# jianglab/helicon

Measured on NVIDIA B200. Metric: denovo3D candidates/sec (solve+score), higher is better.
Workload: dtype f32 (u,v,h) / f64 (x,hbar; bounded branch), as scipy executes it

## Files before the change

helicon_b200/csrc/hb2_api.cu:

```cuda
#include "../../include/helicon_b200.h"
#include "hb2_kernels.cuh"
#include "hb2_trf.cuh"
#include "hb2_symm.cuh"
#include "hb2_tie.cuh"
#include "hb2_fwd_band.cuh"
#include "hb2_adj_tile.cuh"
#include "hb2_explicit.cuh"
#include "hb2_bilinear.cuh"

#include <cub/cub.cuh>
#include <nvtx3/nvToolsExt.h>

#include <algorithm>
#include <cstdio>
#include <cstring>
#include <cstdlib>
#include <string>
#include <vector>

struct NvtxRange {
  explicit NvtxRange(const char* name) { nvtxRangePushA(name); }
  ~NvtxRange() { nvtxRangePop(); }
  NvtxRange(const NvtxRange&) = delete;
  NvtxRange& operator=(const NvtxRange&) = delete;
// ... 190 lines not shown
  float* d_ls_w = nullptr;
  uint16_t* d_amap_i = nullptr;
  bool bilinear = false;
  int bil_nM = 0;
  std::vector<uint8_t> h_bil_rv;
  std::vector<int> h_bil_view_map, h_bil_colk, h_bil_cand_nview;
  std::vector<double> h_bil_ab;
  std::vector<int2*> ls_ent_c;
  std::vector<int> ls_m_c;
  struct LsScratch {
    long long cap_rows = 0, sort_cap = 0;
    int pairs_cap = 0;
    LsymPair* pairs = nullptr;
    unsigned long long *tab_key = nullptr, *tab_seq = nullptr;
    int *tmp_a = nullptr, *tmp_b = nullptr, *flag = nullptr, *pos = nullptr, *ov = nullptr;
    void* scan_tmp = nullptr; size_t scan_bytes = 0;
    int *col = nullptr; float* w = nullptr;
    int *key = nullptr, *key2 = nullptr, *id = nullptr, *id2 = nullptr, *cc = nullptr;
    void* sort_tmp = nullptr; size_t sort_bytes = 0;
  } ls_scr;
  long long extra_launches = 0;
  int max_views = 0;
  bool created = false;
  int nviews = 0;
  std::vector<hb2_candidate> cands;
  std::vector<int> h_view_count, h_view_begin, h_mdata, h_msym;
  std::vector<long long> h_uoff, h_symoff, h_symcap, h_cscoff;
  std::vector<int> tie_per_angle;
  std::vector<int> h_view_angle;
  std::vector<double> h_cs;
  std::vector<uint32_t> cand_flags;
  long long u_total = 0;
  double* d_cs = nullptr;
  void* d_fmap = nullptr;
  uint8_t* d_rayvalid = nullptr;
  int* d_tie = nullptr;
  uint16_t* d_amap = nullptr;
  int* d_sym_g = nullptr;
  std::vector<std::vector<int>> h_sym_round_end;
  int* d_sym_a = nullptr; int* d_sym_b = nullptr; int* d_csc_ptr = nullptr; int* d_csc_ent = nullptr; int* d_ell = nullptr;
  float* d_bmax = nullptr;
  float* d_score = nullptr;
  float* d_chain = nullptr;
  int* d_nactive = nullptr;
  int* h_nactive = nullptr;
  double timing[16] = {0};
  std::vector<TrfState> last_trf;
  std::vector<cudaEvent_t> ev_pool;
  std::vector<std::pair<int, int>> ev_used;
  size_t ev_next = 0;
  bool profiling = false;
  bool solved = false;
  cudaStream_t side = nullptr;
  cudaEvent_t ev_fork = nullptr, ev_join = nullptr;
};

extern "C" const char* hb2_last_error(void) { return g_err.c_str(); }
extern "C" int hb2_device_count(void) {
  int n = 0;
  if (cudaGetDeviceCount(&n) != cudaSuccess) { cudaGetLastError(); return 0; }
  return n;
}
extern "C" const char* hb2_build_info(void) { return "helicon_b200 sm_100a " __DATE__ " " __TIME__; }

extern "C" int hb2_stream_create(int device, void** out) {
  if (!out) return fail(HB2_ERR_ARG, "null argument");
  if (hb2_device_count() <= 0) return fail(HB2_ERR_NO_DEVICE, "no CUDA device visible; helicon_b200 has no CPU fallback");
  CK(cudaSetDevice(device));
  cudaStream_t st;
  CK(cudaStreamCreateWithFlags(&st, cudaStreamNonBlocking));
  *out = (void*)st;
  return HB2_OK;
}
extern "C" int hb2_stream_destroy(int device, void* stream) {
  if (!stream) return HB2_OK;
  CK(cudaSetDevice(device));
  CK(cudaStreamSynchronize((cudaStream_t)stream));
  {
    std::lock_guard<std::mutex> lk(g_arena_mu);
    auto it = g_arenas.find({device, (cudaStream_t)stream});
    if (it != g_arenas.end() && it->second->live == 0) {
      if (it->second->base) cudaFree(it->second->base);
      delete it->second;
      g_arenas.erase(it);
    }
  }
  CK(cudaStreamDestroy((cudaStream_t)stream));
  return HB2_OK;
}
extern "C" int hb2_device_trim(int device) {
  if (hb2_device_count() <= 0) return HB2_OK;
  CK(cudaSetDevice(device));
  CK(cudaDeviceSynchronize());
  std::lock_guard<std::mutex> lk(g_arena_mu);
  for (auto& kv : g_arenas) {
    Arena* a = kv.second;
    if (kv.first.first == device && a->live == 0 && a->base) { cudaFree(a->base); a->base = nullptr; a->cap = 0; a->top = 0; }
  }
  return HB2_OK;
}

static void disk_tables(int G, double rmin, int rmax, std::vector<int>& rank, std::vector<short2>& yx) {
  rank.assign((size_t)G * G, -1);
  yx.clear();
  int c0 = G / 2;
  for (int y = 0; y < G; ++y)
// ... 1447 lines not shown
  ~ProfScope() {
    if (!b->profiling) return;
    cudaEventRecord(b->ev_pool[first + 1], s);
  }
};

static void launch_fwd_data(hb2_batch* b, int mode) {
  ProfScope ps(b, KC_FWD_DATA);
  const BD& B = b->B;
  cudaStream_t st = b->stream;
  if (b->nviews == 0) return;
  if (b->n_tie_views > 0) {
    const float* src = mode == MODE_LSMR ? B.v : B.xs;
    if (b->bilinear) {
      const dim3 gv(b->n_tie_views, B.fwd_ppv);
#define FBIL(I, Q) k_fwd_bil<I, Q, float, false><<<gv, HB2_BLOCK, 0, st>>>(B, TD{}, src, B.u, mode)
#define FBILQ(I) do { if (B.L3P == 4) FBIL(I, 1); else if (B.L3P == 8) FBIL(I, 2); else if (B.L3P == 12) FBIL(I, 3); else FBIL(I, 4); } while (0)
      if (b->idx16) FBILQ(uint16_t); else FBILQ(uint32_t);
#undef FBILQ
#undef FBIL
      k_fwd_lsym<float, false><<<gv, HB2_BLOCK, 0, st>>>(B, TD{}, src, B.u, mode);
      b->extra_launches += 1;
    } else if (b->explicit_rows) k_fwd_csr<float, false><<<dim3(b->n_tie_views, B.fwd_ppv), HB2_BLOCK, 0, st>>>(B, TD{}, src, B.u, mode);
    else if (b->idx16) k_fwd_tie<uint16_t, float, false><<<dim3(b->n_tie_views, B.fwd_ppv), HB2_BLOCK, 0, st>>>(B, TD{}, src, B.u, mode);
    else k_fwd_tie<uint32_t, float, false><<<dim3(b->n_tie_views, B.fwd_ppv), HB2_BLOCK, 0, st>>>(B, TD{}, src, B.u, mode);
    b->extra_launches += 1;
  }
  if (B.fwd_band) {
    const size_t sm = b->fwd_band_smem;
    const dim3 gb(B.bt32.nband, B.nc), gr(b->max_views, B.nc);
#define FWB(Q)                                                                                            \
  do {                                                                                                    \
    hb2_allow_big_smem((const void*)k_fwd_band<Q, float, false>);                                         \
    k_fwd_band<Q, float, false><<<gb, HB2_FWDB_THREADS, sm, st>>>(B, TD{}, nullptr, mode);                \
    k_fwd_band_reduce<Q, float, false><<<gr, HB2_BLOCK, 0, st>>>(B, TD{}, nullptr, mode);                 \
  } while (0)
    if (B.L3P == 4) FWB(1); else if (B.L3P == 8) FWB(2); else if (B.L3P == 12) FWB(3); else FWB(4);
    b->extra_launches += 1;
#undef FWB
    return;
  }
  const int ntiles = (B.D2 + HB2_TILE_RAYS - 1) / HB2_TILE_RAYS;
  unsigned grid = (unsigned)b->nviews * ntiles;
#define FWD(T)                                                                              \
  do {                                                                                      \
    if (B.L3P == 4) k_fwd_data<T, 1><<<grid, HB2_BLOCK, 0, st>>>(B, mode);                  \
    else if (B.L3P == 8) k_fwd_data<T, 2><<<grid, HB2_BLOCK, 0, st>>>(B, mode);             \
    else if (B.L3P == 12) k_fwd_data<T, 3><<<grid, HB2_BLOCK, 0, st>>>(B, mode);            \
    else k_fwd_data<T, 4><<<grid, HB2_BLOCK, 0, st>>>(B, mode);                             \
  } while (0)
  if (b->idx16) FWD(uint16_t); else FWD(uint32_t);
#undef FWD
}
static void launch_fwd_sym(hb2_batch* b, int mode, cudaStream_t on = nullptr) {
  ProfScope ps(b, KC_FWD_SYM, on);
  const BD& B = b->B;
  dim3 g(B.part_us_per_cand, B.nc);
  k_fwd_sym<<<g, HB2_BLOCK, 0, on ? on : b->stream>>>(B, mode);
}
static void launch_adj(hb2_batch* b, int mode) {
  ProfScope ps(b, KC_ADJ);
  const BD& B = b->B;
  dim3 g(B.part_v_per_cand, B.nc);
  cudaStream_t st = b->stream;
  if (b->n_tie_views > 0) {
    if (b->bilinear) {
      const dim3 ga(cdiv(B.ndisk, (HB2_BLOCK / 32) * (32 / (B.L3P / 4))), B.nc);
      const size_t smt = (size_t)HB2_BILT_NS * HB2_BILT_SV * ((size_t)B.bil_KB * HB2_BLOCK * 6 + (size_t)B.bil_rmax * B.L3P * sizeof(float));
      const bool use_tile = B.bil_adj_tile && smt <= 200 * 1024;
#define ABIL(Q)                                                                                      \
  do {                                                                                               \
    k_bil_unblend<Q, float, false><<<b->n_tie_views, HB2_BLOCK, 0, st>>>(B, TD{}, B.u, B.bil_ub, mode); \
    if (use_tile && B.bil_KB == 3) {                                                                 \
      hb2_allow_big_smem((const void*)k_adj_bil_tile<Q, 3, float, false>);                           \
      k_adj_bil_tile<Q, 3, float, false><<<dim3(B.ntile, B.nc), HB2_BILT_THREADS, smt, st>>>(B, TD{}, B.bil_ub, B.vtie, mode); \
    } else if (use_tile) {                                                                           \
      hb2_allow_big_smem((const void*)k_adj_bil_tile<Q, 0, float, false>);                           \
      k_adj_bil_tile<Q, 0, float, false><<<dim3(B.ntile, B.nc), HB2_BILT_THREADS, smt, st>>>(B, TD{}, B.bil_ub, B.vtie, mode); \
    } else k_adj_bil<Q, float, false><<<ga, HB2_BLOCK, 0, st>>>(B, TD{}, B.bil_ub, B.vtie, mode);   \
  } while (0)
      if (B.L3P == 4) ABIL(1); else if (B.L3P == 8) ABIL(2); else if (B.L3P == 12) ABIL(3); else ABIL(4);
#undef ABIL
      k_adj_lsym<float, false><<<dim3(cdiv(B.npad, HB2_BLOCK), B.nc), HB2_BLOCK, 0, st>>>(B, TD{}, B.u, B.vtie, mode);
      b->extra_launches += 2;
    } else if (b->explicit_rows) k_adj_csc<float, false><<<dim3(cdiv(B.npad, HB2_BLOCK / 32), B.nc), HB2_BLOCK, 0, st>>>(B, TD{}, B.u, B.vtie, mode);
    else k_adj_tie<float, false><<<dim3(cdiv(B.ndisk, HB2_BLOCK), B.nc), HB2_BLOCK, 0, st>>>(B, TD{}, B.u, B.vtie, mode);
    b->extra_launches += 1;
  }
  if (B.adj_tile == 2) {
    const size_t sm = b->adj_tile_smem;
    const dim3 gc(B.ntile, B.nc, b->adj_chunks);
#define ADJTC(K)                                                                                                        \
  do {                                                                                                                  \
    hb2_allow_big_smem((const void*)k_adj_tile<4, K, float, false, true>);   \
    k_adj_tile<4, K, float, false, true><<<gc, HB2_ADJT_THREADS, sm, st>>>(B, TD{}, B.u, nullptr, mode);                \
  } while (0)
    if (B.K == 1) ADJTC(1); else ADJTC(2);
#undef ADJTC
    return;
  }
  if (B.adj_tile) {
    const size_t sm = b->adj_tile_smem;
#define ADJT(Q, K)                                                                                                   \
  do {                                                                                                               \
    hb2_allow_big_smem((const void*)k_adj_tile<Q, K, float, false>);      \
    k_adj_tile<Q, K, float, false><<<g, HB2_ADJT_THREADS, sm, st>>>(B, TD{}, B.u, nullptr, mode);                    \
  } while (0)
#define ADJTQ(K) do { if (B.L3P == 4) ADJT(1, K); else if (B.L3P == 8) ADJT(2, K); else if (B.L3P == 12) ADJT(3, K); else ADJT(4, K); } while (0)
    if (B.K == 1) ADJTQ(1); else ADJTQ(2);
#undef ADJTQ
#undef ADJT
    return;
  }
  if (B.adj_fast) {
    if (B.K == 1) k_adj_pq<1><<<g, HB2_BLOCK, 0, st>>>(B, mode);
    else k_adj_pq<2><<<g, HB2_BLOCK, 0, st>>>(B, mode);
    return;
  }
#define ADJ(K, M) k_adj<K, M><<<g, HB2_BLOCK, 0, st>>>(B, mode)
  if (B.MC == 1) ADJ(0, 1);
  else ADJ(0, 0);
#undef ADJ
}
static void launch_update(hb2_batch* b, int mode) {
  ProfScope ps(b, KC_UPDATE);
  const BD& B = b->B;
  dim3 g(B.part_x_per_cand, B.nc);
  k_update<<<g, HB2_BLOCK, 0, b->stream>>>(B, mode);
}

extern "C" int hb2_batch_apply_forward(hb2_batch* b, int32_t c, const float* x_host, float* y_host) {
  if (!b || !b->created || !x_host || !y_host || c < 0 || c >= b->B.nc) return fail(HB2_ERR_ARG, "bad argument");
  CK(cudaSetDevice(b->P->device));
  BD& B = b->B;
  cudaStream_t st = b->stream;
  long long m = (long long)b->h_mdata[c] + b->h_msym[c];
  std::vector<float> xi((size_t)B.npad, 0.f);
  for (int z = 0; z < B.L3; ++z)
    for (int pp = 0; pp < B.ndisk; ++pp) xi[(size_t)pp * B.L3P + z] = x_host[(size_t)z * B.ndisk + b->P->int2ref[pp]];
  CK(cudaMemcpyAsync(B.xs + (size_t)c * B.npad, xi.data(), sizeof(float) * B.npad, cudaMemcpyHostToDevice, st));
  CK(cudaMemsetAsync(B.u + b->h_uoff[c], 0, sizeof(float) * m, st));
  B.only_cand = c;
  launch_fwd_data(b, MODE_PLAIN);
  launch_fwd_sym(b, MODE_PLAIN);
  B.only_cand = -1;
  CKL();
  CK(cudaMemcpyAsync(y_host, B.u + b->h_uoff[c], sizeof(float) * m, cudaMemcpyDeviceToHost, st));
  CK(cudaStreamSynchronize(st));
  b->solved = false;
  return HB2_OK;
}

extern "C" int hb2_batch_apply_adjoint(hb2_batch* b, int32_t c, const float* y_host, float* x_host) {
  if (!b || !b->created || !x_host || !y_host || c < 0 || c >= b->B.nc) return fail(HB2_ERR_ARG, "bad argument");
  CK(cudaSetDevice(b->P->device));
  BD& B = b->B;
  cudaStream_t st = b->stream;
  long long m = (long long)b->h_mdata[c] + b->h_msym[c];
  CK(cudaMemcpyAsync(B.u + b->h_uoff[c], y_host, sizeof(float) * m, cudaMemcpyHostToDevice, st));
  B.only_cand = c;
  launch_adj(b, MODE_PLAIN);
  B.only_cand = -1;
  CKL();
  std::vector<float> xi((size_t)B.npad);
  CK(cudaMemcpyAsync(xi.data(), B.xs + (size_t)c * B.npad, sizeof(float) * B.npad, cudaMemcpyDeviceToHost, st));
  CK(cudaStreamSynchronize(st));
  for (int z = 0; z < B.L3; ++z)
    for (int pp = 0; pp < B.ndisk; ++pp) x_host[(size_t)z * B.ndisk + b->P->int2ref[pp]] = xi[(size_t)pp * B.L3P + z];
  b->solved = false;
  return HB2_OK;
}


static int run_trf(hb2_batch* b, const hb2_solve_options* opt, std::vector<TrfState>& out, long long& launches, int& outer_iters) {
  BD& B = b->B;
  cudaStream_t st = b->stream;
  const int nc = B.nc;
  bool any = false;
  for (int c = 0; c < nc; ++c) any = any || b->cands[c].positive;
  out.assign(nc, TrfState{});
  if (!any) return HB2_OK;
// ... 172 lines not shown
  }
  pass(OPC(EW_FINAL));
#undef OPC
  CKT2(cudaGetLastError());
  CKT2(cudaMemcpyAsync(out.data(), T.st, sizeof(TrfState) * nc, cudaMemcpyDeviceToHost, st));
  CKT2(cudaStreamSynchronize(st));
  tmp.free_all();
  B.vtie64 = nullptr;
  return HB2_OK;
}

extern "C" int hb2_batch_solve(hb2_batch* b, const hb2_solve_options* opt, hb2_result* res) {
  if (!b || !b->created || !opt || !res) return fail(HB2_ERR_ARG, "bad argument");
  CK(cudaSetDevice(b->P->device));
  NvtxRange nvtx_("solve_equations + score (batch)");
  nvtxRangePushA("solve_equations: LSMR");
  struct PopGuard { int n = 1; ~PopGuard() { while (n-- > 0) nvtxRangePop(); } } nvtx_stage_;
  BD& B = b->B;
  cudaStream_t st = b->stream;
  const int nc = B.nc;
  const int maxit = opt->max_iter > 0 ? opt->max_iter : 1000;
  const int check = opt->check_every > 0 ? opt->check_every : 8;
  B.clip_pred = opt->clip_pred;
  B.only_cand = -1;
  b->profiling = opt->profile != 0;
  b->ev_used.clear();
  b->ev_next = 0;
  cudaEvent_t e0, e1, e2;
  CK(cudaEventCreate(&e0)); CK(cudaEventCreate(&e1)); CK(cudaEventCreate(&e2));
  CK(cudaEventRecord(e0, st));
  size_t nv = (size_t)nc * B.npad;
  CK(cudaMemsetAsync(B.x, 0, nv * sizeof(double), st));
  CK(cudaMemsetAsync(B.hbar, 0, nv * sizeof(double), st));
  CK(cudaMemsetAsync(B.h, 0, nv * sizeof(float), st));
  CK(cudaMemsetAsync(B.v, 0, nv * sizeof(float), st));
  CK(cudaMemcpyAsync(B.u, B.b, sizeof(float) * (size_t)b->u_total, cudaMemcpyDeviceToDevice, st));
  CK(cudaMemsetAsync(b->d_nactive, 0, sizeof(int), st));
  long long launches = 0;
  b->extra_launches = 0;
  static const int env_norm = [] { const char* e = getenv("HB2_NORM_MODE"); return e ? atoi(e) : -1; }();
  const bool chain = (env_norm >= 0 ? env_norm : opt->norm_mode) != 0;
  if (chain) {
    hb2_allow_big_smem((const void*)k_chain_sumsq<CHAIN_U>);
    hb2_allow_big_smem((const void*)k_chain_sumsq<CHAIN_V>);
    hb2_allow_big_smem((const void*)k_chain_sumsq<CHAIN_B>);
  }
  float* ch_u = chain ? b->d_chain : nullptr;
  float* ch_v = chain ? b->d_chain + nc : nullptr;
  if (chain) { k_chain_sumsq<CHAIN_B><<<nc, 64, HB2_CHAIN_SMEM, st>>>(B, ch_u, MODE_INIT); ++launches; }
  k_scal_normb<<<nc, HB2_BLOCK, 0, st>>>(B, ch_u);
  launch_adj(b, MODE_INIT);
  if (chain) { k_chain_sumsq<CHAIN_V><<<nc, 64, HB2_CHAIN_SMEM, st>>>(B, ch_v, MODE_INIT); ++launches; }
  k_scal_init<<<nc, HB2_BLOCK, 0, st>>>(B, b->d_nactive, ch_v);
  launch_update(b, MODE_INIT);
  launches += 4;
  CKL();
  int it = 0;
  static const int env_overlap = [] { const char* e = getenv("HB2_OVERLAP"); return e ? atoi(e) : 1; }();
  const bool overlap = env_overlap != 0 && !b->profiling;
  if (overlap && !b->side) {
    CK(cudaStreamCreateWithFlags(&b->side, cudaStreamNonBlocking));
    CK(cudaEventCreateWithFlags(&b->ev_fork, cudaEventDisableTiming));
    CK(cudaEventCreateWithFlags(&b->ev_join, cudaEventDisableTiming));
  }
  *b->h_nactive = 1;
  CK(cudaMemcpyAsync(b->h_nactive, b->d_nactive, sizeof(int), cudaMemcpyDeviceToHost, st));
  CK(cudaStreamSynchronize(st));
  while (*b->h_nactive > 0 && it < maxit) {
    int burst = std::min(check, maxit - it);
    for (int q = 0; q < burst; ++q) {
      if (overlap) {
        cudaEventRecord(b->ev_fork, st);
        launch_fwd_data(b, MODE_LSMR);
        cudaStreamWaitEvent(b->side, b->ev_fork, 0);
        launch_fwd_sym(b, MODE_LSMR, b->side);
        cudaEventRecord(b->ev_join, b->side);
        cudaStreamWaitEvent(st, b->ev_join, 0);
      } else {
        launch_fwd_data(b, MODE_LSMR);
        launch_fwd_sym(b, MODE_LSMR);
      }
      if (chain) { ProfScope ps(b, KC_NORM); k_chain_sumsq<CHAIN_U><<<nc, 64, HB2_CHAIN_SMEM, st>>>(B, ch_u, MODE_LSMR); ++launches; }
      { ProfScope ps(b, KC_SCALAR); k_scal_beta<<<nc, HB2_BLOCK, 0, st>>>(B, ch_u); }
      launch_adj(b, MODE_LSMR);
      if (chain) { ProfScope ps(b, KC_NORM); k_chain_sumsq<CHAIN_V><<<nc, 64, HB2_CHAIN_SMEM, st>>>(B, ch_v, MODE_LSMR); ++launches; }
      { ProfScope ps(b, KC_SCALAR); k_scal_rot<<<nc, HB2_BLOCK, 0, st>>>(B, ch_v); }
      launch_update(b, MODE_LSMR);
      { ProfScope ps(b, KC_SCALAR); k_scal_test<<<nc, HB2_BLOCK, 0, st>>>(B, opt->atol, opt->btol, opt->conlim, maxit, opt->fixed_iters, b->d_nactive); }
      launches += 7;
    }
    it += burst;
    CKL();
    CK(cudaMemcpyAsync(b->h_nactive, b->d_nactive, sizeof(int), cudaMemcpyDeviceToHost, st));
    CK(cudaStreamSynchronize(st));
  }
  CK(cudaEventRecord(e1, st));
  std::vector<TrfState> trf;
  int trf_outer = 0;
  cudaEvent_t e1b;
  CK(cudaEventCreate(&e1b));
  {
    dim3 g(cdiv(B.npad, 256), nc);
    k_x_to_f32<<<g, 256, 0, st>>>(B);
    ++launches;
  }
  nvtxRangePop(); nvtxRangePushA("solve_equations: bounded TRF");
  if (opt->fixed_iters <= 0) {
    int rc = run_trf(b, opt, trf, launches, trf_outer);
    if (rc != HB2_OK) return rc;
  } else trf.assign(nc, TrfState{});
  CK(cudaEventRecord(e1b, st));
  nvtxRangePop(); nvtxRangePushA("cosine_similarity (reprojection + score)");
  {
    launch_fwd_data(b, MODE_SCORE);
    k_scal_score<<<nc, HB2_BLOCK, 0, st>>>(B, b->d_score);
    launches += 2;
    CKL();
  }
  CK(cudaEventRecord(e2, st));
  std::vector<LsmrState> hs(nc);
  std::vector<float> sc(nc);
  CK(cudaMemcpyAsync(hs.data(), B.st, sizeof(LsmrState) * nc, cudaMemcpyDeviceToHost, st));
  CK(cudaMemcpyAsync(sc.data(), b->d_score, sizeof(float) * nc, cudaMemcpyDeviceToHost, st));
  CK(cudaStreamSynchronize(st));
  float ms_l = 0, ms_s = 0, ms_t = 0;
  cudaEventElapsedTime(&ms_l, e0, e1); cudaEventElapsedTime(&ms_t, e1, e1b); cudaEventElapsedTime(&ms_s, e1b, e2);
  cudaEventDestroy(e0); cudaEventDestroy(e1); cudaEventDestroy(e1b); cudaEventDestroy(e2);
  for (double& t : b->timing) t = 0;
  b->timing[0] = ms_l; b->timing[1] = ms_t; b->timing[2] = ms_s; b->timing[13] = trf_outer; b->timing[3] = (double)(launches + b->extra_launches); b->timing[4] = it;
  if (b->profiling) {
    for (auto& pr : b->ev_used) {
      float ms = 0;
      cudaEventElapsedTime(&ms, b->ev_pool[pr.second], b->ev_pool[pr.second + 1]);
      if (pr.first == KC_NORM) b->timing[14] += ms;
      else b->timing[5 + pr.first] += ms;
      if (pr.first == KC_FWD_DATA) b->timing[10] += 1;
      if (pr.first == KC_ADJ) b->timing[11] += 1;
      if (pr.first == KC_UPDATE) b->timing[12] += 1;
    }
    b->profiling = false;
  }
  for (int c = 0; c < nc; ++c) {
    hb2_result& r = res[c];
// ... 319 lines not shown
```

helicon_b200/csrc/hb2_kernels.cuh:

```cuda
#pragma once
#include "hb2_common.cuh"

#define HB2_MAX_ZMC 1024
#define HB2_TILE_RAYS 32
#define HB2_BLOCK 256
#define HB2_FWD_U 8
#define HB2_ELL_W 4
#define HB2_MAXDUP 3
#define HB2_ELL_NONE 0x7FFFFFFF
#define HB2_ELL_OVERFLOW 0x7FFFFFFE

enum { MODE_LSMR = 0, MODE_PLAIN = 1, MODE_SCORE = 2, MODE_INIT = 3 };

struct BandTab {
  int nband;
  const int* band_begin;
  const ushort2* seg;
  const ushort2* rng;
  const int* band_off;
  const long long* view_poff;
  void* part;
};

struct BD {
// ... 917 lines not shown
    for (int tz = 0; tz < 4; ++tz) {
      float s2 = a2[tz];
      if (ev[HB2_ELL_W - 1][tz] == HB2_ELL_OVERFLOW) {
        const int* __restrict__ ptr = B.csc_ptr + (size_t)c * (B.npad + 1) + g0 + tz;
        const int* __restrict__ ent = B.csc_ent + B.cand_cscoff[c];
        for (int e = ptr[0]; e < ptr[1]; ++e) {
          const int x = ent[e];
          const float val = __ldg(us + (x & 0x7fffffff));
          s2 = fmaf(x < 0 ? -val : val, ib, s2);
        }
      } else {
#pragma unroll
        for (int w = 0; w < HB2_ELL_W; ++w)
          if (ev[w][tz] != HB2_ELL_NONE) s2 = fmaf(ev[w][tz] < 0 ? -vals[w][tz] : vals[w][tz], ib, s2);
      }
      const float o = tz == 0 ? old.x : (tz == 1 ? old.y : (tz == 2 ? old.z : old.w));
      vn[tz] = mode == MODE_LSMR ? fadd_(fmul_(o, -beta), s2) : s2;
      ss += vn[tz] * vn[tz];
    }
    *reinterpret_cast<float4*>(vdst) = make_float4(vn[0], vn[1], vn[2], vn[3]);
  }
  if (mode != MODE_PLAIN) {
    float tot = block_sum(ss, red);
    if (threadIdx.x == 0) B.part_v[pi] = tot;
  }
}

__global__ void __launch_bounds__(HB2_BLOCK) k_tile_rays(int K, int apitch, int ntile, const uint16_t* __restrict__ amap,
                                                        uint16_t* __restrict__ jlo, uint16_t* __restrict__ nr,
                                                        int* __restrict__ rmax) {
  const int t = blockIdx.x, a = blockIdx.y;
  __shared__ int s_lo[HB2_BLOCK / 32], s_hi[HB2_BLOCK / 32];
  int lo = 0x7fffffff, hi = -1;
  for (int k = 0; k < K; ++k) {
    const unsigned j = amap[((size_t)a * K + k) * apitch + (size_t)t * HB2_BLOCK + threadIdx.x];
    if (j != 0xFFFFu) { lo = min(lo, (int)j); hi = max(hi, (int)j); }
  }
#pragma unroll
  for (int o = 16; o > 0; o >>= 1) {
    lo = min(lo, __shfl_xor_sync(0xffffffffu, lo, o));
    hi = max(hi, __shfl_xor_sync(0xffffffffu, hi, o));
  }
  if ((threadIdx.x & 31) == 0) { s_lo[threadIdx.x >> 5] = lo; s_hi[threadIdx.x >> 5] = hi; }
  __syncthreads();
  if (threadIdx.x == 0) {
    for (int w = 1; w < HB2_BLOCK / 32; ++w) { lo = min(lo, s_lo[w]); hi = max(hi, s_hi[w]); }
    const int n = hi >= 0 ? hi - lo + 1 : 0;
    jlo[(size_t)a * ntile + t] = (uint16_t)(n ? lo : 0);
    nr[(size_t)a * ntile + t] = (uint16_t)n;
    if (n) atomicMax(rmax, n);
  }
}

__global__ void __launch_bounds__(HB2_BLOCK) k_update(BD B, int mode) {
  const int c = blockIdx.y;
  __shared__ double redd[HB2_BLOCK / 32];
  const LsmrState& S = B.st[c];
  const int pi = c * B.part_x_per_cand + blockIdx.x;
  if (!S.active) {
    if (threadIdx.x == 0) B.part_x[pi] = 0.0;
    return;
  }
  const float ia = S.inv_alpha;
  const double cfhb = (double)S.cf_hbar, cfx = (double)S.cf_x;
  const float cfh = S.cf_h;
  const bool normalise = !(mode == MODE_LSMR && S.skip_adj);
  float4* v4 = reinterpret_cast<float4*>(B.v + (size_t)c * B.npad);
  float4* h4 = reinterpret_cast<float4*>(B.h + (size_t)c * B.npad);
  double2* x2 = reinterpret_cast<double2*>(B.x + (size_t)c * B.npad);
  double2* hb2 = reinterpret_cast<double2*>(B.hbar + (size_t)c * B.npad);
  const int n4 = B.npad >> 2;
  double sx = 0.0;
  const int i = blockIdx.x * HB2_BLOCK + threadIdx.x;
  if (i < n4) {
    float4 vq = v4[i];
    float vn[4] = {vq.x, vq.y, vq.z, vq.w};
    if (normalise) {
#pragma unroll
      for (int k = 0; k < 4; ++k) vn[k] = fmul_(vn[k], ia);
      v4[i] = make_float4(vn[0], vn[1], vn[2], vn[3]);
    }
    if (mode == MODE_INIT) {
      h4[i] = make_float4(vn[0], vn[1], vn[2], vn[3]);
      hb2[2 * i] = make_double2(0.0, 0.0); hb2[2 * i + 1] = make_double2(0.0, 0.0);
      x2[2 * i] = make_double2(0.0, 0.0); x2[2 * i + 1] = make_double2(0.0, 0.0);
    } else {
      const float4 hq = h4[i];
      const float ho[4] = {hq.x, hq.y, hq.z, hq.w};
      const double2 b0 = hb2[2 * i], b1 = hb2[2 * i + 1];
      const double2 x0 = x2[2 * i], x1 = x2[2 * i + 1];
      double hb[4] = {b0.x, b0.y, b1.x, b1.y};
      double xn[4] = {x0.x, x0.y, x1.x, x1.y};
      float hn[4];
#pragma unroll
      for (int k = 0; k < 4; ++k) {
        hb[k] = dadd_(dmul_(hb[k], cfhb), (double)ho[k]);
        xn[k] = dadd_(xn[k], dmul_(cfx, hb[k]));
        hn[k] = fadd_(fmul_(ho[k], cfh), vn[k]);
        sx += xn[k] * xn[k];
      }
      hb2[2 * i] = make_double2(hb[0], hb[1]); hb2[2 * i + 1] = make_double2(hb[2], hb[3]);
      x2[2 * i] = make_double2(xn[0], xn[1]); x2[2 * i + 1] = make_double2(xn[2], xn[3]);
      h4[i] = make_float4(hn[0], hn[1], hn[2], hn[3]);
    }
  }
  double tot = block_sum_d(sx, redd);
  if (threadIdx.x == 0) B.part_x[pi] = tot;
}

__global__ void k_x_to_f32(BD B) {
  const int c = blockIdx.y;
  int i = blockIdx.x * blockDim.x + threadIdx.x;
  if (i < B.npad) B.xs[(size_t)c * B.npad + i] = (float)B.x[(size_t)c * B.npad + i];
}

__device__ __forceinline__ double reduce_partials_f(const float* p, int n, double* shd) {
  double s = 0.0;
  for (int i = threadIdx.x; i < n; i += HB2_BLOCK) s += (double)p[i];
  return block_sum_d(s, shd);
}

#define HB2_CHAIN_STAGES 6
#define HB2_CHAIN_STAGE_F4 1024
#define HB2_CHAIN_SMEM (HB2_CHAIN_STAGES * HB2_CHAIN_STAGE_F4 * 16)
enum { CHAIN_U = 0, CHAIN_V = 1, CHAIN_B = 2 };
template <int WHICH>
__global__ void __launch_bounds__(64) k_chain_sumsq(BD B, float* __restrict__ out, int mode) {
  const int c = blockIdx.x;
  if (mode == MODE_LSMR && !B.st[c].active) return;
  const float* p;
  long long n;
  if (WHICH == CHAIN_U) { p = B.u + B.cand_uoff[c]; n = (long long)B.cand_mdata[c] + ((B.cand_msym[c] + 3) & ~3); }
  else if (WHICH == CHAIN_V) { p = B.v + (size_t)c * B.npad; n = B.npad; }
  else { p = B.b + B.cand_uoff[c]; n = B.cand_mdata[c]; }
  const float4* __restrict__ p4 = reinterpret_cast<const float4*>(p);
  const long long n4 = n >> 2;
  extern __shared__ __align__(128) unsigned char chain_smem[];
  float4 (*ring)[HB2_CHAIN_STAGE_F4] = reinterpret_cast<float4 (*)[HB2_CHAIN_STAGE_F4]>(chain_smem);
  __shared__ unsigned long long full_bar[HB2_CHAIN_STAGES];
  __shared__ float a[64];
  const int lane = threadIdx.x;
  const long long nstage = (n4 + HB2_CHAIN_STAGE_F4 - 1) / HB2_CHAIN_STAGE_F4;
  if (lane == 0) {
#pragma unroll
    for (int i = 0; i < HB2_CHAIN_STAGES; ++i) mbar_init(&full_bar[i], 1);
  }
  asm volatile("fence.mbarrier_init.release.cluster;\n" ::: "memory");
  __syncthreads();
  auto issue = [&](long long st) {
    const int buf = (int)(st % HB2_CHAIN_STAGES);
    const long long lo = st * HB2_CHAIN_STAGE_F4;
    const unsigned bytes = (unsigned)(min((long long)HB2_CHAIN_STAGE_F4, n4 - lo) * 16);
    mbar_expect_tx(&full_bar[buf], bytes);
    bulk_g2s(&ring[buf][0], p4 + lo, bytes, &full_bar[buf]);
  };
  if (lane == 0)
    for (long long st = 0; st < min((long long)HB2_CHAIN_STAGES - 1, nstage); ++st) issue(st);
  float acc = 0.f;
  for (long long st = 0; st < nstage; ++st) {
    const int buf = (int)(st % HB2_CHAIN_STAGES);
// ... 11 lines not shown
#pragma unroll
    for (int k = 0; k < 16; ++k) {
      acc = __fmaf_rn(t[k].x, t[k].x, acc); acc = __fmaf_rn(t[k].y, t[k].y, acc);
      acc = __fmaf_rn(t[k].z, t[k].z, acc); acc = __fmaf_rn(t[k].w, t[k].w, acc);
    }
    __syncthreads();
  }
  a[lane] = acc;
  __syncthreads();
  if (lane == 0) {
    float a8[8];
#pragma unroll
    for (int l = 0; l < 8; ++l) {
      float q[4];
#pragma unroll
      for (int k = 0; k < 4; ++k) q[k] = fadd_(a[16 * k + l], a[16 * k + l + 8]);
      a8[l] = fadd_(fadd_(fadd_(q[0], q[1]), q[2]), q[3]);
    }
    float h[4];
#pragma unroll
    for (int l = 0; l < 4; ++l) h[l] = fadd_(a8[l], a8[l + 4]);
    out[c] = fadd_(fadd_(h[0], h[1]), fadd_(h[2], h[3]));
  }
}

__global__ void __launch_bounds__(HB2_BLOCK) k_scal_normb(BD B, const float* __restrict__ chain) {
  const int c = blockIdx.x;
  __shared__ double shd[HB2_BLOCK / 32];
  const float* bb = B.b + B.cand_uoff[c];
  double s = 0.0;
  if (!chain) {
    for (int i = threadIdx.x; i < B.cand_mdata[c]; i += HB2_BLOCK) { double t = bb[i]; s += t * t; }
    s = block_sum_d(s, shd);
  }
  if (threadIdx.x == 0) {
    LsmrState& S = B.st[c];
    float beta = __fsqrt_rn(chain ? chain[c] : (float)s);
    S.beta = beta; S.normb = beta;
    S.inv_beta = beta > 0.f ? fdiv_(1.f, beta) : 0.f;
    S.alpha = 0.f; S.active = 1; S.skip_adj = 0; S.istop = 0; S.itn = 0;
  }
}
__global__ void __launch_bounds__(HB2_BLOCK) k_scal_init(BD B, int* nactive, const float* __restrict__ chain) {
  const int c = blockIdx.x;
  __shared__ double shd[HB2_BLOCK / 32];
  double s = chain ? 0.0 : reduce_partials_f(B.part_v + (size_t)c * B.part_v_per_cand, B.part_v_per_cand, shd);
  if (threadIdx.x == 0) {
    LsmrState& S = B.st[c];
    float alpha = __fsqrt_rn(chain ? chain[c] : (float)s);
    lsmr_init_(S, alpha, S.beta);
    if (S.active) atomicAdd(nactive, 1);
  }
}
__global__ void __launch_bounds__(HB2_BLOCK) k_scal_beta(BD B, const float* __restrict__ chain) {
  const int c = blockIdx.x;
  __shared__ double shd[HB2_BLOCK / 32];
  LsmrState& S = B.st[c];
  if (!S.active) return;
  const int ntiles = B.fwd_ppv;
  double s = 0.0;
  if (!chain) {
    s = reduce_partials_f(B.part_u + (size_t)B.cand_view_begin[c] * ntiles, B.cand_view_count[c] * ntiles, shd);
    s += reduce_partials_f(B.part_us + (size_t)c * B.part_us_per_cand, B.part_us_per_cand, shd);
  }
  if (threadIdx.x == 0) {
    float beta = __fsqrt_rn(chain ? chain[c] : (float)s);
    S.beta = beta;
    if (beta > 0.f) { S.inv_beta = fdiv_(1.f, beta); S.skip_adj = 0; }
    else { S.skip_adj = 1; }
  }
}
__global__ void __launch_bounds__(HB2_BLOCK) k_scal_rot(BD B, const float* __restrict__ chain) {
  const int c = blockIdx.x;
  __shared__ double shd[HB2_BLOCK / 32];
  LsmrState& S = B.st[c];
  if (!S.active) return;
  double s = chain ? 0.0 : reduce_partials_f(B.part_v + (size_t)c * B.part_v_per_cand, B.part_v_per_cand, shd);
  if (threadIdx.x == 0) {
    float alpha = S.skip_adj ? S.alpha : __fsqrt_rn(chain ? chain[c] : (float)s);
    lsmr_rotate_(S, alpha, S.beta);
  }
}
__global__ void __launch_bounds__(HB2_BLOCK) k_scal_test(BD B, double atol, double btol, double conlim, int maxiter,
                                                         int fixed_iters, int* nactive) {
  const int c = blockIdx.x;
  __shared__ double shd[HB2_BLOCK / 32];
  LsmrState& S = B.st[c];
  if (!S.active) return;
  double s = 0.0;
  for (int i = threadIdx.x; i < B.part_x_per_cand; i += HB2_BLOCK) s += B.part_x[(size_t)c * B.part_x_per_cand + i];
  s = block_sum_d(s, shd);
  if (threadIdx.x == 0) {
    int istop = lsmr_test_(S, sqrt(s), atol, btol, conlim, maxiter);
    if (fixed_iters > 0) { istop = S.itn >= fixed_iters ? 7 : 0; S.istop = istop; }
    if (istop > 0) { S.active = 0; atomicSub(nactive, 1); }
  }
}
__global__ void __launch_bounds__(HB2_BLOCK) k_scal_score(BD B, float* __restrict__ score) {
  const int c = blockIdx.x;
  __shared__ double shd[HB2_BLOCK / 32];
  const int ntiles = B.fwd_ppv;
  const int n = B.cand_view_count[c] * ntiles;
  const float* p = B.part_s + (size_t)B.cand_view_begin[c] * ntiles * 3;
  double d = 0, pp = 0, bb = 0;
  for (int i = threadIdx.x; i < n; i += HB2_BLOCK) { d += p[3 * i]; pp += p[3 * i + 1]; bb += p[3 * i + 2]; }
  d = block_sum_d(d, shd); pp = block_sum_d(pp, shd); bb = block_sum_d(bb, shd);
  if (threadIdx.x == 0) {
    float na = __fsqrt_rn((float)pp), nb = __fsqrt_rn((float)bb);
    float norm = fmul_(na, nb);
    score[c] = norm == 0.f ? 0.f : fdiv_((float)d, norm);
  }
}
```

profiles/prof_overlap.py:

```python
import os, sys
sys.path.insert(0, os.path.dirname(os.path.dirname(os.path.abspath(__file__))))
import numpy as np
import bench
from helicon_b200.engine import Batch, Problem
from helicon_b200.planner import MAX_EQUATIONS, CandidateSpec

nc = int(sys.argv[1]) if len(sys.argv) > 1 else 100
ni = int(sys.argv[2]) if len(sys.argv) > 2 else 60
img = bench.synthetic_filament()
tasks = bench.grid_tasks()
g = tasks[0].geom
prob = Problem(img, g["s"], g["D2"], g["L2"], g["D3"], 0.0, g["D3"] // 2 - 1)
n3 = g["L3"] * prob.ndisk
target = min(MAX_EQUATIONS, int(max(g["D2"] * g["L2"], n3) * g["sym_oversample"]))
sel = tasks[20000:20000 + nc]
batch = Batch(prob, g["L3"], [CandidateSpec(t.twist, t.rise / g["apix3d"], 1, target, target, False) for t in sel])
for prof in (0, 0, 0, 1):
    res = batch.solve(fixed_iters=ni, check_every=ni, profile=prof)
    tm = batch.timing()
    print(f"HB2_OVERLAP={os.environ.get('HB2_OVERLAP', '1')} profile={prof}: lsmr {tm['lsmr_ms']:.2f} ms = "
          f"{1e3 * tm['lsmr_ms'] / (nc * ni):.2f} us per candidate-iteration; fwd_data {tm['fwd_data_ms']:.1f} fwd_sym "
          f"{tm['fwd_sym_ms']:.1f} adj {tm['adj_ms']:.1f} update {tm['update_ms']:.1f} norm {tm['norm_ms']:.1f}; "
          f"score checksum {float(np.sum(res['score'].astype(np.float64))):.9f}")
batch.close(); prob.close()
```

Measured before the change: 60.95.

## Overlap LSMR x/h recurrence on side stream with next iteration's forward pass

Measured after the change: 58.49, median of 6. -4.0%, worse.

```diff
diff --git a/helicon_b200/csrc/hb2_api.cu b/helicon_b200/csrc/hb2_api.cu
--- a/helicon_b200/csrc/hb2_api.cu
+++ b/helicon_b200/csrc/hb2_api.cu
@@ -266,6 +266,7 @@
   bool profiling = false;
   bool solved = false;
   cudaStream_t side = nullptr;
+  int nsm = 0;
   cudaEvent_t ev_fork = nullptr, ev_join = nullptr;
 };
 
@@ -1819,11 +1820,11 @@
   if (b->idx16) FWD(uint16_t); else FWD(uint32_t);
 #undef FWD
 }
-static void launch_fwd_sym(hb2_batch* b, int mode, cudaStream_t on = nullptr) {
-  ProfScope ps(b, KC_FWD_SYM, on);
+static void launch_fwd_sym(hb2_batch* b, int mode) {
+  ProfScope ps(b, KC_FWD_SYM);
   const BD& B = b->B;
   dim3 g(B.part_us_per_cand, B.nc);
-  k_fwd_sym<<<g, HB2_BLOCK, 0, on ? on : b->stream>>>(B, mode);
+  k_fwd_sym<<<g, HB2_BLOCK, 0, b->stream>>>(B, mode);
 }
 static void launch_adj(hb2_batch* b, int mode) {
   ProfScope ps(b, KC_ADJ);
@@ -1889,11 +1890,16 @@
   else ADJ(0, 0);
 #undef ADJ
 }
-static void launch_update(hb2_batch* b, int mode) {
+static void launch_update(hb2_batch* b, void (*kern)(BD)) {
   ProfScope ps(b, KC_UPDATE);
   const BD& B = b->B;
-  dim3 g(B.part_x_per_cand, B.nc);
-  k_update<<<g, HB2_BLOCK, 0, b->stream>>>(B, mode);
+  kern<<<dim3(B.part_x_per_cand, B.nc), HB2_BLOCK, 0, b->stream>>>(B);
+}
+static void launch_recur(hb2_batch* b, bool side) {
+  ProfScope ps(b, KC_UPDATE, side ? b->side : nullptr);
+  const BD& B = b->B;
+  const int ntile = B.part_x_per_cand * B.nc;
+  k_recur<<<side ? std::min(ntile, b->nsm) : ntile, HB2_BLOCK, 0, side ? b->side : b->stream>>>(B);
 }
 
 extern "C" int hb2_batch_apply_forward(hb2_batch* b, int32_t c, const float* x_host, float* y_host) {
@@ -2172,43 +2178,45 @@
   launch_adj(b, MODE_INIT);
   if (chain) { k_chain_sumsq<CHAIN_V><<<nc, 64, HB2_CHAIN_SMEM, st>>>(B, ch_v, MODE_INIT); ++launches; }
   k_scal_init<<<nc, HB2_BLOCK, 0, st>>>(B, b->d_nactive, ch_v);
-  launch_update(b, MODE_INIT);
+  launch_update(b, k_update_init);
   launches += 4;
   CKL();
   int it = 0;
-  static const int env_overlap = [] { const char* e = getenv("HB2_OVERLAP"); return e ? atoi(e) : 1; }();
-  const bool overlap = env_overlap != 0 && !b->profiling;
+  const char* env_overlap = getenv("HB2_OVERLAP");
+  const bool overlap = !env_overlap || atoi(env_overlap) != 0;
   if (overlap && !b->side) {
+    CK(cudaDeviceGetAttribute(&b->nsm, cudaDevAttrMultiProcessorCount, b->P->device));
     CK(cudaStreamCreateWithFlags(&b->side, cudaStreamNonBlocking));
     CK(cudaEventCreateWithFlags(&b->ev_fork, cudaEventDisableTiming));
     CK(cudaEventCreateWithFlags(&b->ev_join, cudaEventDisableTiming));
   }
+  const StopTest tst{opt->atol, opt->btol, opt->conlim, maxit, opt->fixed_iters, b->d_nactive};
   *b->h_nactive = 1;
   CK(cudaMemcpyAsync(b->h_nactive, b->d_nactive, sizeof(int), cudaMemcpyDeviceToHost, st));
   CK(cudaStreamSynchronize(st));
   while (*b->h_nactive > 0 && it < maxit) {
     int burst = std::min(check, maxit - it);
     for (int q = 0; q < burst; ++q) {
-      if (overlap) {
-        cudaEventRecord(b->ev_fork, st);
-        launch_fwd_data(b, MODE_LSMR);
-        cudaStreamWaitEvent(b->side, b->ev_fork, 0);
-        launch_fwd_sym(b, MODE_LSMR, b->side);
-        cudaEventRecord(b->ev_join, b->side);
-        cudaStreamWaitEvent(st, b->ev_join, 0);
-      } else {
-        launch_fwd_data(b, MODE_LSMR);
-        launch_fwd_sym(b, MODE_LSMR);
-      }
+      launch_fwd_data(b, MODE_LSMR);
+      launch_fwd_sym(b, MODE_LSMR);
+      if (overlap && q > 0) cudaStreamWaitEvent(st, b->ev_join, 0);
       if (chain) { ProfScope ps(b, KC_NORM); k_chain_sumsq<CHAIN_U><<<nc, 64, HB2_CHAIN_SMEM, st>>>(B, ch_u, MODE_LSMR); ++launches; }
-      { ProfScope ps(b, KC_SCALAR); k_scal_beta<<<nc, HB2_BLOCK, 0, st>>>(B, ch_u); }
+      { ProfScope ps(b, KC_SCALAR); k_scal_beta<<<nc, HB2_BLOCK, 0, st>>>(B, ch_u, q > 0, tst); }
       launch_adj(b, MODE_LSMR);
       if (chain) { ProfScope ps(b, KC_NORM); k_chain_sumsq<CHAIN_V><<<nc, 64, HB2_CHAIN_SMEM, st>>>(B, ch_v, MODE_LSMR); ++launches; }
       { ProfScope ps(b, KC_SCALAR); k_scal_rot<<<nc, HB2_BLOCK, 0, st>>>(B, ch_v); }
-      launch_update(b, MODE_LSMR);
-      { ProfScope ps(b, KC_SCALAR); k_scal_test<<<nc, HB2_BLOCK, 0, st>>>(B, opt->atol, opt->btol, opt->conlim, maxit, opt->fixed_iters, b->d_nactive); }
+      launch_update(b, k_norm_v);
+      if (overlap) {
+        cudaEventRecord(b->ev_fork, st);
+        cudaStreamWaitEvent(b->side, b->ev_fork, 0);
+      }
+      launch_recur(b, overlap);
+      if (overlap) cudaEventRecord(b->ev_join, b->side);
       launches += 7;
     }
+    if (overlap) cudaStreamWaitEvent(st, b->ev_join, 0);
+    { ProfScope ps(b, KC_SCALAR); k_scal_test<<<nc, HB2_BLOCK, 0, st>>>(B, tst); }
+    ++launches;
     it += burst;
     CKL();
     CK(cudaMemcpyAsync(b->h_nactive, b->d_nactive, sizeof(int), cudaMemcpyDeviceToHost, st));
diff --git a/helicon_b200/csrc/hb2_kernels.cuh b/helicon_b200/csrc/hb2_kernels.cuh
--- a/helicon_b200/csrc/hb2_kernels.cuh
+++ b/helicon_b200/csrc/hb2_kernels.cuh
@@ -993,40 +993,61 @@
   }
 }
 
-__global__ void __launch_bounds__(HB2_BLOCK) k_update(BD B, int mode) {
+__global__ void __launch_bounds__(HB2_BLOCK) k_update_init(BD B) {
   const int c = blockIdx.y;
-  __shared__ double redd[HB2_BLOCK / 32];
   const LsmrState& S = B.st[c];
-  const int pi = c * B.part_x_per_cand + blockIdx.x;
-  if (!S.active) {
-    if (threadIdx.x == 0) B.part_x[pi] = 0.0;
-    return;
-  }
+  if (threadIdx.x == 0) B.part_x[c * B.part_x_per_cand + blockIdx.x] = 0.0;
+  if (!S.active) return;
   const float ia = S.inv_alpha;
-  const double cfhb = (double)S.cf_hbar, cfx = (double)S.cf_x;
-  const float cfh = S.cf_h;
-  const bool normalise = !(mode == MODE_LSMR && S.skip_adj);
   float4* v4 = reinterpret_cast<float4*>(B.v + (size_t)c * B.npad);
   float4* h4 = reinterpret_cast<float4*>(B.h + (size_t)c * B.npad);
   double2* x2 = reinterpret_cast<double2*>(B.x + (size_t)c * B.npad);
   double2* hb2 = reinterpret_cast<double2*>(B.hbar + (size_t)c * B.npad);
-  const int n4 = B.npad >> 2;
-  double sx = 0.0;
   const int i = blockIdx.x * HB2_BLOCK + threadIdx.x;
-  if (i < n4) {
-    float4 vq = v4[i];
-    float vn[4] = {vq.x, vq.y, vq.z, vq.w};
-    if (normalise) {
-#pragma unroll
-      for (int k = 0; k < 4; ++k) vn[k] = fmul_(vn[k], ia);
-      v4[i] = make_float4(vn[0], vn[1], vn[2], vn[3]);
-    }
-    if (mode == MODE_INIT) {
-      h4[i] = make_float4(vn[0], vn[1], vn[2], vn[3]);
-      hb2[2 * i] = make_double2(0.0, 0.0); hb2[2 * i + 1] = make_double2(0.0, 0.0);
-      x2[2 * i] = make_double2(0.0, 0.0); x2[2 * i + 1] = make_double2(0.0, 0.0);
-    } else {
-      const float4 hq = h4[i];
+  if (i < (B.npad >> 2)) {
+    const float4 vq = v4[i];
+    const float4 vn = make_float4(fmul_(vq.x, ia), fmul_(vq.y, ia), fmul_(vq.z, ia), fmul_(vq.w, ia));
+    v4[i] = vn;
+    h4[i] = vn;
+    hb2[2 * i] = make_double2(0.0, 0.0); hb2[2 * i + 1] = make_double2(0.0, 0.0);
+    x2[2 * i] = make_double2(0.0, 0.0); x2[2 * i + 1] = make_double2(0.0, 0.0);
+  }
+}
+
+__global__ void __launch_bounds__(HB2_BLOCK) k_norm_v(BD B) {
+  const int c = blockIdx.y;
+  const LsmrState& S = B.st[c];
+  if (!S.active || S.skip_adj) return;
+  const float ia = S.inv_alpha;
+  float4* v4 = reinterpret_cast<float4*>(B.v + (size_t)c * B.npad);
+  const int i = blockIdx.x * HB2_BLOCK + threadIdx.x;
+  if (i < (B.npad >> 2)) {
+    const float4 vq = v4[i];
+    v4[i] = make_float4(fmul_(vq.x, ia), fmul_(vq.y, ia), fmul_(vq.z, ia), fmul_(vq.w, ia));
+  }
+}
+
+__global__ void __launch_bounds__(HB2_BLOCK, 5) k_recur(BD B) {
+  __shared__ double redd[HB2_BLOCK / 32];
+  const int ppc = B.part_x_per_cand, ntile = ppc * B.nc;
+  for (int t = blockIdx.x; t < ntile; t += gridDim.x) {
+    const int c = t / ppc;
+    const LsmrState& S = B.st[c];
+    if (!S.active) {
+      if (threadIdx.x == 0) B.part_x[t] = 0.0;
+      continue;
+    }
+    const double cfhb = (double)S.cf_hbar, cfx = (double)S.cf_x;
+    const float cfh = S.cf_h;
+    const float4* v4 = reinterpret_cast<const float4*>(B.v + (size_t)c * B.npad);
+    float4* h4 = reinterpret_cast<float4*>(B.h + (size_t)c * B.npad);
+    double2* x2 = reinterpret_cast<double2*>(B.x + (size_t)c * B.npad);
+    double2* hb2 = reinterpret_cast<double2*>(B.hbar + (size_t)c * B.npad);
+    double sx = 0.0;
+    const int i = (t - c * ppc) * HB2_BLOCK + threadIdx.x;
+    if (i < (B.npad >> 2)) {
+      const float4 vq = v4[i], hq = h4[i];
+      const float vn[4] = {vq.x, vq.y, vq.z, vq.w};
       const float ho[4] = {hq.x, hq.y, hq.z, hq.w};
       const double2 b0 = hb2[2 * i], b1 = hb2[2 * i + 1];
       const double2 x0 = x2[2 * i], x1 = x2[2 * i + 1];
@@ -1044,9 +1065,9 @@
       x2[2 * i] = make_double2(xn[0], xn[1]); x2[2 * i + 1] = make_double2(xn[2], xn[3]);
       h4[i] = make_float4(hn[0], hn[1], hn[2], hn[3]);
     }
-  }
-  double tot = block_sum_d(sx, redd);
-  if (threadIdx.x == 0) B.part_x[pi] = tot;
+    double tot = block_sum_d(sx, redd);
+    if (threadIdx.x == 0) B.part_x[t] = tot;
+  }
 }
 
 __global__ void k_x_to_f32(BD B) {
@@ -1164,11 +1185,32 @@
     if (S.active) atomicAdd(nactive, 1);
   }
 }
-__global__ void __launch_bounds__(HB2_BLOCK) k_scal_beta(BD B, const float* __restrict__ chain) {
+struct StopTest {
+  double atol, btol, conlim;
+  int maxiter, fixed_iters;
+  int* nactive;
+};
+__device__ __forceinline__ bool stop_test_(BD& B, int c, const StopTest& t, double* shd) {
+  __shared__ int s_stop;
+  LsmrState& S = B.st[c];
+  double s = 0.0;
+  for (int i = threadIdx.x; i < B.part_x_per_cand; i += HB2_BLOCK) s += B.part_x[(size_t)c * B.part_x_per_cand + i];
+  s = block_sum_d(s, shd);
+  if (threadIdx.x == 0) {
+    int istop = lsmr_test_(S, sqrt(s), t.atol, t.btol, t.conlim, t.maxiter);
+    if (t.fixed_iters > 0) { istop = S.itn >= t.fixed_iters ? 7 : 0; S.istop = istop; }
+    if (istop > 0) { S.active = 0; atomicSub(t.nactive, 1); }
+    s_stop = istop > 0;
+  }
+  __syncthreads();
+  return s_stop != 0;
+}
+__global__ void __launch_bounds__(HB2_BLOCK) k_scal_beta(BD B, const float* __restrict__ chain, int test, StopTest t) {
   const int c = blockIdx.x;
   __shared__ double shd[HB2_BLOCK / 32];
   LsmrState& S = B.st[c];
   if (!S.active) return;
+  if (test && stop_test_(B, c, t, shd)) return;
   const int ntiles = B.fwd_ppv;
   double s = 0.0;
   if (!chain) {
@@ -1193,20 +1235,11 @@
     lsmr_rotate_(S, alpha, S.beta);
   }
 }
-__global__ void __launch_bounds__(HB2_BLOCK) k_scal_test(BD B, double atol, double btol, double conlim, int maxiter,
-                                                         int fixed_iters, int* nactive) {
+__global__ void __launch_bounds__(HB2_BLOCK) k_scal_test(BD B, StopTest t) {
   const int c = blockIdx.x;
   __shared__ double shd[HB2_BLOCK / 32];
-  LsmrState& S = B.st[c];
-  if (!S.active) return;
-  double s = 0.0;
-  for (int i = threadIdx.x; i < B.part_x_per_cand; i += HB2_BLOCK) s += B.part_x[(size_t)c * B.part_x_per_cand + i];
-  s = block_sum_d(s, shd);
-  if (threadIdx.x == 0) {
-    int istop = lsmr_test_(S, sqrt(s), atol, btol, conlim, maxiter);
-    if (fixed_iters > 0) { istop = S.itn >= fixed_iters ? 7 : 0; S.istop = istop; }
-    if (istop > 0) { S.active = 0; atomicSub(nactive, 1); }
-  }
+  if (!B.st[c].active) return;
+  stop_test_(B, c, t, shd);
 }
 __global__ void __launch_bounds__(HB2_BLOCK) k_scal_score(BD B, float* __restrict__ score) {
   const int c = blockIdx.x;
diff --git a/profiles/prof_overlap.py b/profiles/prof_overlap.py
--- a/profiles/prof_overlap.py
+++ b/profiles/prof_overlap.py
@@ -1,25 +1,71 @@
-import os, sys
-sys.path.insert(0, os.path.dirname(os.path.dirname(os.path.abspath(__file__))))
-import numpy as np
-import bench
-from helicon_b200.engine import Batch, Problem
-from helicon_b200.planner import MAX_EQUATIONS, CandidateSpec
+import argparse, json, os, subprocess, sys
 
-nc = int(sys.argv[1]) if len(sys.argv) > 1 else 100
-ni = int(sys.argv[2]) if len(sys.argv) > 2 else 60
-img = bench.synthetic_filament()
-tasks = bench.grid_tasks()
-g = tasks[0].geom
-prob = Problem(img, g["s"], g["D2"], g["L2"], g["D3"], 0.0, g["D3"] // 2 - 1)
-n3 = g["L3"] * prob.ndisk
-target = min(MAX_EQUATIONS, int(max(g["D2"] * g["L2"], n3) * g["sym_oversample"]))
-sel = tasks[20000:20000 + nc]
-batch = Batch(prob, g["L3"], [CandidateSpec(t.twist, t.rise / g["apix3d"], 1, target, target, False) for t in sel])
-for prof in (0, 0, 0, 1):
-    res = batch.solve(fixed_iters=ni, check_every=ni, profile=prof)
-    tm = batch.timing()
-    print(f"HB2_OVERLAP={os.environ.get('HB2_OVERLAP', '1')} profile={prof}: lsmr {tm['lsmr_ms']:.2f} ms = "
-          f"{1e3 * tm['lsmr_ms'] / (nc * ni):.2f} us per candidate-iteration; fwd_data {tm['fwd_data_ms']:.1f} fwd_sym "
-          f"{tm['fwd_sym_ms']:.1f} adj {tm['adj_ms']:.1f} update {tm['update_ms']:.1f} norm {tm['norm_ms']:.1f}; "
-          f"score checksum {float(np.sum(res['score'].astype(np.float64))):.9f}")
-batch.close(); prob.close()
+ROOT = os.path.dirname(os.path.dirname(os.path.abspath(__file__)))
+ARMS = {"serial": {"HB2_OVERLAP": "0"}, "overlap": {"HB2_OVERLAP": "1"}}
+CLASSES = ("fwd_data_ms", "fwd_sym_ms", "adj_ms", "update_ms", "scalar_ms", "norm_ms")
+
+
+def run_arm(nc, ni, reps):
+    sys.path.insert(0, ROOT)
+    import numpy as np
+    import bench
+    from helicon_b200.engine import Batch, Problem
+    from helicon_b200.planner import MAX_EQUATIONS, CandidateSpec
+
+    img = bench.synthetic_filament()
+    tasks = bench.grid_tasks()
+    g = tasks[0].geom
+    prob = Problem(img, g["s"], g["D2"], g["L2"], g["D3"], 0.0, g["D3"] // 2 - 1)
+    n3 = g["L3"] * prob.ndisk
+    target = min(MAX_EQUATIONS, int(max(g["D2"] * g["L2"], n3) * g["sym_oversample"]))
+    sel = tasks[20000:20000 + nc]
+    batch = Batch(prob, g["L3"], [CandidateSpec(t.twist, t.rise / g["apix3d"], 1, target, target, False) for t in sel])
+    batch.solve(fixed_iters=ni, check_every=ni, profile=0)
+    out = {}
+    for prof in (0, 1):
+        us, sums = [], set()
+        for _ in range(reps):
+            res = batch.solve(fixed_iters=ni, check_every=ni, profile=prof)
+            tm = batch.timing()
+            us.append(1e3 * tm["lsmr_ms"] / (nc * ni))
+            sums.add(float(np.sum(res["score"].astype(np.float64))))
+        out[f"profile{prof}"] = dict(us_per_cand_iter_median=float(np.median(us)), us_per_cand_iter=us,
+                                     score_checksum=sorted(sums))
+        if prof:
+            out["profile1"]["class_us_per_cand_iter"] = {k: 1e3 * tm[k] / (nc * ni) for k in CLASSES}
+    batch.close(); prob.close()
+    return out
+
+
+def main():
+    ap = argparse.ArgumentParser()
+    ap.add_argument("nc", type=int, nargs="?", default=200)
+    ap.add_argument("ni", type=int, nargs="?", default=60)
+    ap.add_argument("--reps", type=int, default=5)
+    ap.add_argument("--out", default=None)
+    ap.add_argument("--arm", default=None, help=argparse.SUPPRESS)
+    a = ap.parse_args()
+    if a.arm:
+        print(json.dumps(run_arm(a.nc, a.ni, a.reps)))
+        return
+    smi = subprocess.run(["nvidia-smi", "--query-gpu=name,power.limit,clocks.sm,clocks.max.sm", "--format=csv,noheader"],
+                         capture_output=True, text=True).stdout.strip()
+    result = dict(gpu_power_limit_sm_clock_max_sm_clock=smi, candidates=a.nc, iterations=a.ni, reps=a.reps, arms={})
+    for name, env in ARMS.items():
+        p = subprocess.run([sys.executable, os.path.abspath(__file__), str(a.nc), str(a.ni), "--reps", str(a.reps),
+                            "--arm", name], env={**os.environ, **env}, capture_output=True, text=True, cwd=ROOT)
+        if p.returncode != 0:
+            sys.exit(f"arm {name} failed:\n{p.stderr[-4000:]}")
+        result["arms"][name] = json.loads(p.stdout.strip().splitlines()[-1])
+        r = result["arms"][name]
+        print(f"{name}: profile0 {r['profile0']['us_per_cand_iter_median']:.2f} us, profile1 "
+              f"{r['profile1']['us_per_cand_iter_median']:.2f} us per candidate-iteration; score checksum "
+              f"{r['profile0']['score_checksum']}", flush=True)
+    if a.out:
+        with open(a.out, "w") as f:
+            json.dump(result, f, indent=1)
+    print(json.dumps(result))
+
+
+if __name__ == "__main__":
+    main()
```
